# ShunyaoWang/quadruped_locomotion

Hardware: NVIDIA B200
Metric: contact-force QPs solved/sec (higher is better)
Workload: dtype f64

## Files before the change

### quadruped_locomotion_b200/csrc/qlb_api.cu

```cuda
#include <cuda_runtime.h>
#include <dlfcn.h>
#include <nccl.h>

#include <cmath>
#include <cstdio>
#include <cstdlib>
#include <cstring>
#include <mutex>
#include <new>

#include "qlb.h"
#include "qlb_aux.cuh"
#include "qlb_gen.cuh"
#include "qlb_qp_dense.cuh"
#include "qlb_records.cuh"
#include "qlb_solve.cuh"
#include "qlb_solve_quad.cuh"
#include "qlb_solve_fused.cuh"
#include "qlb_solve_single.cuh"
#include "qlb_swing.cuh"
#include "qlb_tick.cuh"

using namespace qlb;

// ... 141 lines not shown
    }
    const double* R3 = m->rot[l][3];
    const double* c3 = legs[l].link_com[3];
    for (int a = 0; a < 3; a++) m->com[l][3][a] = R3[3 * a] * c3[0] + R3[3 * a + 1] * c3[1] + R3[3 * a + 2] * c3[2];
    double acc = 0.0;
    for (int j = 3; j >= 0; j--) { acc += legs[l].link_mass[j]; m->msuf[l][j] = acc; }
  }
}

void build_device_params(const qlb_params* p, DeviceParams* d) {
  std::memset(d, 0, sizeof *d);
  for (int i = 0; i < 6; i++) d->S[i] = p->wrench_weights[i];
  d->W = p->ground_force_weight;
  d->fmin = p->min_normal_force > 0.0 ? p->min_normal_force : 0.0;
  d->mu_default = p->friction_default;
  d->gravity = p->gravity;
  d->tol = p->ipm_tolerance;
  d->max_iter = p->ipm_max_iterations;
  for (int i = 0; i < 3; i++) {
    d->kp_t[i] = p->kp_translation[i]; d->kd_t[i] = p->kd_translation[i]; d->kff_t[i] = p->kff_translation[i];
    d->kp_r[i] = p->kp_rotation[i]; d->kd_r[i] = p->kd_rotation[i]; d->kff_r[i] = p->kff_rotation[i];
    d->com[i] = p->com_in_base[i];
  }
  d->torso_mass = p->torso_mass;
  for (int l = 0; l < 4; l++) {
    d->leg_mass[l] = p->leg_mass[l];
    for (int a = 0; a < 3; a++) d->leg_pos[l][a] = p->leg_base_position[l][a];
  }
  d->grav_pct = p->gravity_compensation_percentage;
}

void narrow_model(const DeviceModel& m, DeviceModelT<float>* f) {
  const double* src = reinterpret_cast<const double*>(&m);
  float* dst = reinterpret_cast<float*>(f);
  for (size_t i = 0; i < sizeof(DeviceModel) / sizeof(double); i++) dst[i] = (float)src[i];
}
void narrow_params(const DeviceParams& d, DeviceParamsT<float>* f) {
  std::memset(f, 0, sizeof *f);
  for (int i = 0; i < 6; i++) f->S[i] = (float)d.S[i];
  f->W = (float)d.W; f->fmin = (float)d.fmin; f->mu_default = (float)d.mu_default; f->gravity = (float)d.gravity;
  f->tol = (float)d.tol; f->max_iter = d.max_iter;
  for (int i = 0; i < 3; i++) {
    f->kp_t[i] = (float)d.kp_t[i]; f->kd_t[i] = (float)d.kd_t[i]; f->kff_t[i] = (float)d.kff_t[i];
    f->kp_r[i] = (float)d.kp_r[i]; f->kd_r[i] = (float)d.kd_r[i]; f->kff_r[i] = (float)d.kff_r[i];
    f->com[i] = (float)d.com[i];
  }
  f->torso_mass = (float)d.torso_mass;
  for (int l = 0; l < 4; l++) {
    f->leg_mass[l] = (float)d.leg_mass[l];
    for (int a = 0; a < 3; a++) f->leg_pos[l][a] = (float)d.leg_pos[l][a];
  }
  f->grav_pct = (float)d.grav_pct;
}

bool params_ok(const qlb_params* p) {
  const double lo = 1e-12, hi = 1e12;
  if (!(p->ground_force_weight >= lo && p->ground_force_weight <= hi) || !(p->ipm_tolerance > 0.0) || p->ipm_max_iterations < 1)
    return false;
  for (int i = 0; i < 6; i++)
    if (!(p->wrench_weights[i] >= lo && p->wrench_weights[i] <= hi)) return false;
  if (!(p->friction_default >= 0.0) || !std::isfinite(p->friction_default)) return false;
  if (!(std::fabs(p->min_normal_force) <= 1e9)) return false;
  return std::isfinite(p->gravity);
}

bool aligned16(const void* p) { return (reinterpret_cast<uintptr_t>(p) & 15u) == 0; }

template <typename T>
int prepare_slot(qlb_context* ctx, SolveArgsT<T>& a, cudaStream_t st) {
  if (a.B > 0xFFFFFFF0ull) return QLB_ERR_BATCH_TOO_LARGE;
  int slot = -1;
  for (int i = 0; i < 8 && slot < 0; i++)
    if (cudaEventQuery(ctx->slot_done[i]) == cudaSuccess) slot = i;
  cudaGetLastError();
  if (slot < 0) slot = (int)(ctx->solve_calls % 8);
  ctx->solve_calls++;
  ctx->last_slot = slot;
  QLB_CUDA(ctx, cudaStreamWaitEvent(st, ctx->slot_done[slot], 0));
  a.counter = ctx->d_counter + 8 * slot;
  a.counter2 = a.counter + 1;
  a.counter3 = a.counter + 2;
  a.list_count = reinterpret_cast<unsigned*>(a.counter + 3);
  a.list2_count = reinterpret_cast<unsigned*>(a.counter + 4);
  QLB_CUDA(ctx, cudaMemsetAsync(a.counter, 0, 8 * sizeof(unsigned long long), st));
  if (ctx->list_cap < a.B) {
    const size_t cap = pow2_at_least(a.B, 1024);
    ctx->list_cap = 0;
    QLB_TRY(reserve(ctx, ctx->lists, 8 * 3 * cap * sizeof(unsigned)));
    ctx->list_cap = cap;
  }
  unsigned* list = reinterpret_cast<unsigned*>(ctx->lists.p) + (size_t)slot * 3 * ctx->list_cap;
  a.list = list;
  a.list2 = list + ctx->list_cap;
  a.list_pat = list + 2 * ctx->list_cap;
  return QLB_OK;
}

template <typename T, typename C>
constexpr int occ_index() { return sizeof(T) == 8 ? 0 : sizeof(C) == 8 ? 1 : 2; }

template <typename T, typename C, int MODE>
int launch_quad(qlb_context* ctx, SolveArgsT<T>& a, cudaStream_t st) {
  const SolveOccupancy& occ = ctx->occ[occ_index<T, C>()];
  const unsigned long long nb8 = (a.B + 7) / 8;
  const unsigned long long wantq = (nb8 + (kQuadThreads / 32) - 1) / (kQuadThreads / 32);
  const unsigned long long capq = (unsigned long long)ctx->sm_count * occ.quad[MODE];
  const unsigned long long capf = (unsigned long long)ctx->sm_count * occ.first[MODE];
  const unsigned gq = (unsigned)(wantq < capq ? wantq : capq);
  qlb_quad_first_kernel<T, C, MODE><<<(unsigned)(wantq < capf ? wantq : capf), kQuadThreads, 0, st>>>(a);
  QLB_CUDA(ctx, cudaGetLastError());
  ctx->launches++;
  qlb_quad_kernel<T, C, MODE, 1><<<gq, kQuadThreads, 0, st>>>(a);
  QLB_CUDA(ctx, cudaGetLastError());
  ctx->launches++;
  qlb_quad_kernel<T, C, MODE, 2><<<gq, kQuadThreads, 0, st>>>(a);
  QLB_CUDA(ctx, cudaGetLastError());
  ctx->launches++;
  QLB_CUDA(ctx, cudaEventRecord(ctx->slot_done[ctx->last_slot], st));
  return QLB_OK;
}

typedef CUresult (*EncodeTiledFn)(CUtensorMap*, CUtensorMapDataType, cuuint32_t, void*, const cuuint64_t*, const cuuint64_t*,
                                  const cuuint32_t*, const cuuint32_t*, CUtensorMapInterleave, CUtensorMapSwizzle,
                                  CUtensorMapL2promotion, CUtensorMapFloatOOBfill);
EncodeTiledFn encode_tiled_fn() {
  static EncodeTiledFn fn = []() -> EncodeTiledFn {
    void* p = nullptr;
    cudaDriverEntryPointQueryResult qres;
    if (cudaGetDriverEntryPoint("cuTensorMapEncodeTiled", &p, cudaEnableDefault, &qres) != cudaSuccess || qres != cudaDriverEntryPointSuccess) {
      cudaGetLastError();
      return nullptr;
    }
    return reinterpret_cast<EncodeTiledFn>(p);
  }();
  return fn;
}

template <typename T>
bool make_map(CUtensorMap* m, const T* ptr, unsigned long long B, int rows) {
  EncodeTiledFn fn = encode_tiled_fn();
  if (!fn) return false;
  const cuuint64_t gdim[2] = {(cuuint64_t)B, (cuuint64_t)rows};
  const cuuint64_t gstride[1] = {(cuuint64_t)B * sizeof(T)};
  const cuuint32_t box[2] = {8u * QLB_SUPER, (cuuint32_t)rows};
  const cuuint32_t estr[2] = {1u, 1u};
  return fn(m, sizeof(T) == 8 ? CU_TENSOR_MAP_DATA_TYPE_FLOAT64 : CU_TENSOR_MAP_DATA_TYPE_FLOAT32, 2, const_cast<T*>(ptr), gdim,
            gstride, box, estr, CU_TENSOR_MAP_INTERLEAVE_NONE, CU_TENSOR_MAP_SWIZZLE_NONE, CU_TENSOR_MAP_L2_PROMOTION_L2_128B,
            CU_TENSOR_MAP_FLOAT_OOB_FILL_NONE) == CUDA_SUCCESS;
}

bool make_mask_map(CUtensorMap* m, const uint8_t* ptr, unsigned long long B, int cols) {
  EncodeTiledFn fn = encode_tiled_fn();
  if (!fn) return false;
  const cuuint64_t gdim[1] = {(cuuint64_t)B};
  const cuuint64_t gstride[1] = {0};
  const cuuint32_t box[1] = {(cuuint32_t)cols};
  const cuuint32_t estr[1] = {1u};
  return fn(m, CU_TENSOR_MAP_DATA_TYPE_UINT8, 1, const_cast<uint8_t*>(ptr), gdim, gstride, box, estr, CU_TENSOR_MAP_INTERLEAVE_NONE,
            CU_TENSOR_MAP_SWIZZLE_NONE, CU_TENSOR_MAP_L2_PROMOTION_NONE, CU_TENSOR_MAP_FLOAT_OOB_FILL_NONE) == CUDA_SUCCESS;
}

template <typename T, typename C, int MODE>
int launch_single(qlb_context* ctx, SolveArgsT<T>& a, cudaStream_t st) {
  const SolveOccupancy& occ = ctx->occ[occ_index<T, C>()];
  using SG = Staging<T, MODE, QLB_SUPER>;
  using FL = FusedLayout<T, C, MODE, QLB_SUPER>;
  const T* src[SG::kNumSeg];
  for (int s = 0; s < SG::kNumSeg; s++) src[s] = SG::source(a, s);
  bool tma = a.B >= 64 && a.B < 0x7fffff00ull && ((a.B * sizeof(T)) % 16 == 0);
  for (int s = 0; s < SG::kNumSeg && tma; s++)
    if (src[s] && !aligned16(src[s])) tma = false;
  FusedMaps maps;
  std::memset(&maps, 0, sizeof maps);
  for (int s = 0; s < SG::kNumSeg && tma; s++)
    if (src[s] && !make_map<T>(&maps.seg[s], src[s], a.B, SG::rows(s))) tma = false;
  if (tma && (SG::kCols < 16 || !aligned16(a.mask) || !make_mask_map(&maps.mask, a.mask, a.B, SG::kCols))) tma = false;
  const unsigned long long ntiles = (a.B + 7) / 8;
  const unsigned long long want = (ntiles + kFusedWarps - 1) / kFusedWarps;
  int bps = occ.single[MODE][tma ? 1 : 0];
  if (ctx->fused_bps_cap > 0 && bps > ctx->fused_bps_cap) bps = ctx->fused_bps_cap;
  const unsigned long long cap = (unsigned long long)ctx->sm_count * bps;
  const unsigned grid = (unsigned)(want < cap ? want : cap);
  if (tma) qlb_single_kernel<T, C, MODE, QLB_SUPER, true><<<grid, kFusedThreads, FL::kTotal, st>>>(a, maps);
  else qlb_single_kernel<T, C, MODE, QLB_SUPER, false><<<grid, kFusedThreads, FL::kTotal, st>>>(a, maps);
  QLB_CUDA(ctx, cudaGetLastError());
  ctx->launches++;
  const unsigned long long capq = (unsigned long long)ctx->sm_count * occ.quad[MODE];
  const unsigned long long wantq = (ntiles + 3) / 4;
  qlb_quad_kernel<T, C, MODE, 2><<<(unsigned)(wantq < capq ? wantq : capq), kQuadThreads, 0, st>>>(a);
  QLB_CUDA(ctx, cudaGetLastError());
  ctx->launches++;
  QLB_CUDA(ctx, cudaEventRecord(ctx->slot_done[ctx->last_slot], st));
  return QLB_OK;
}

template <typename T, typename C>
bool query_occupancy(qlb_context* ctx) {
  SolveOccupancy& o = ctx->occ[occ_index<T, C>()];
  if (cudaOccupancyMaxActiveBlocksPerMultiprocessor(&o.quad[0], qlb_quad_kernel<T, C, 0, 2>, kQuadThreads, 0) != cudaSuccess ||
      cudaOccupancyMaxActiveBlocksPerMultiprocessor(&o.quad[1], qlb_quad_kernel<T, C, 1, 2>, kQuadThreads, 0) != cudaSuccess ||
      cudaOccupancyMaxActiveBlocksPerMultiprocessor(&o.first[0], qlb_quad_first_kernel<T, C, 0>, kQuadThreads, 0) != cudaSuccess ||
      cudaOccupancyMaxActiveBlocksPerMultiprocessor(&o.first[1], qlb_quad_first_kernel<T, C, 1>, kQuadThreads, 0) != cudaSuccess)
    return false;
  return o.quad[0] >= 1 && o.quad[1] >= 1 && o.first[0] >= 1 && o.first[1] >= 1;
}

template <typename T, int MODE>
bool prepare_single_kernels(qlb_context* ctx) {
  using C = double;
  using FL = FusedLayout<T, C, MODE, QLB_SUPER>;
  int* out = ctx->occ[occ_index<T, C>()].single[MODE];
  if (cudaFuncSetAttribute(qlb_single_kernel<T, C, MODE, QLB_SUPER, false>, cudaFuncAttributeMaxDynamicSharedMemorySize, FL::kTotal) != cudaSuccess ||
      cudaFuncSetAttribute(qlb_single_kernel<T, C, MODE, QLB_SUPER, true>, cudaFuncAttributeMaxDynamicSharedMemorySize, FL::kTotal) != cudaSuccess ||
      cudaFuncSetAttribute(qlb_single_kernel<T, C, MODE, QLB_SUPER, false>, cudaFuncAttributePreferredSharedMemoryCarveout, cudaSharedmemCarveoutMaxShared) != cudaSuccess ||
      cudaFuncSetAttribute(qlb_single_kernel<T, C, MODE, QLB_SUPER, true>, cudaFuncAttributePreferredSharedMemoryCarveout, cudaSharedmemCarveoutMaxShared) != cudaSuccess)
    return false;
  if (cudaOccupancyMaxActiveBlocksPerMultiprocessor(&out[0], qlb_single_kernel<T, C, MODE, QLB_SUPER, false>, kFusedThreads, FL::kTotal) != cudaSuccess ||
      cudaOccupancyMaxActiveBlocksPerMultiprocessor(&out[1], qlb_single_kernel<T, C, MODE, QLB_SUPER, true>, kFusedThreads, FL::kTotal) != cudaSuccess)
    return false;
  return out[0] >= 1 && out[1] >= 1;
}

template <typename T, int MODE>
int launch_solve(qlb_context* ctx, SolveArgsT<T>& a, cudaStream_t st) {
  QLB_TRY(prepare_slot(ctx, a, st));
  if constexpr (sizeof(T) == 4) {
    if (ctx->f32_pure) return launch_quad<float, float, MODE>(ctx, a, st);
  }
  if (ctx->pipeline == QLB_PIPELINE_FUSED) return launch_single<T, double, MODE>(ctx, a, st);
  return launch_quad<T, double, MODE>(ctx, a, st);
}

constexpr size_t kSoaBytesPerState = (kHostInRows + kHostOutRows) * sizeof(double) + sizeof(uint32_t) + 1;
struct SoaSlot {
  double* in;
  double* out;
  uint32_t* flags;
  uint8_t* mask;
};
SoaSlot soa_slot(const qlb_context* ctx, int slot) {
  const size_t cap = ctx->cap;
  double* in = reinterpret_cast<double*>(ctx->soa.p);
  double* out = in + kPipe * cap * kHostInRows;
  uint32_t* flags = reinterpret_cast<uint32_t*>(out + kPipe * cap * kHostOutRows);
  uint8_t* mask = reinterpret_cast<uint8_t*>(flags + kPipe * cap);
  return {in + slot * cap * kHostInRows, out + slot * cap * kHostOutRows, flags + slot * cap, mask + slot * cap};
}

int reserve_soa(qlb_context* ctx, size_t B) {
  if (B > kChunk) B = kChunk;
  if (B <= ctx->cap) return QLB_OK;
  const size_t cap = pow2_at_least(B, ctx->cap ? ctx->cap : 1024);
  ctx->cap = 0;
  QLB_TRY(reserve(ctx, ctx->soa, kPipe * cap * kSoaBytesPerState));
  ctx->cap = cap;
  return QLB_OK;
}

template <typename F>
int for_chunks(qlb_context* ctx, size_t B, size_t chunk, bool pipelined, F&& body) {
  cudaStream_t* streams = pipelined ? ctx->pipe : &ctx->stream;
  const int nstreams = pipelined ? kPipe : 1;
  int used = 0, rc = QLB_OK;
  for (size_t b0 = 0, i = 0; b0 < B && rc == QLB_OK; b0 += chunk, i++) {
    const int slot = (int)(i % nstreams);
    if (used <= slot) {
      used = slot + 1;
      const cudaError_t e = cudaStreamWaitEvent(streams[slot], ctx->soa_free, 0);
      if (e != cudaSuccess) { rc = cuda_fail(ctx, e, "cudaStreamWaitEvent"); break; }
    }
    rc = body(b0, B - b0 < chunk ? B - b0 : chunk, slot, streams[slot]);
  }
// ... 141 lines not shown
  while (*c) {
    const char* eol = c;
    while (*eol && *eol != '\n') eol++;
    int indent = 0;
    const char* t = c;
    while (t < eol && *t == ' ') { indent++; t++; }
    const char* hash = t;
    while (hash < eol && *hash != '#') hash++;
    const char* end = hash;
    while (end > t && (end[-1] == ' ' || end[-1] == '\t' || end[-1] == '\r')) end--;
    if (end > t && *t != '-') {
      const char* colon = t;
      while (colon < end && *colon != ':') colon++;
      if (colon < end) {
        while (depth > 0 && stack[depth - 1].indent >= indent) depth--;
        plen = depth > 0 ? stack[depth - 1].len : 0;
        const size_t klen = (size_t)(colon - t);
        if (plen + 1 + klen + 1 < sizeof path && depth < 32) {
          path[plen] = '/';
          std::memcpy(path + plen + 1, t, klen);
          const size_t nlen = plen + 1 + klen;
          path[nlen] = 0;
          const char* v = colon + 1;
          while (v < end && *v == ' ') v++;
          if (v < end) {
            char buf[64];
            const size_t vl = (size_t)(end - v) < sizeof buf - 1 ? (size_t)(end - v) : sizeof buf - 1;
            std::memcpy(buf, v, vl);
            buf[vl] = 0;
            char* stop = nullptr;
            const double val = std::strtod(buf, &stop);
            if (stop != buf) {
              const int k = qlb_params_set_key(p, path, val);
              if (k >= 0) seen[k] = true;
            }
          } else {
            stack[depth].indent = indent; stack[depth].len = nlen; depth++;
          }
        }
      }
    }
    c = *eol ? eol + 1 : eol;
  }
  int found = 0;
  const char* miss = nullptr;
  for (int k = 0; k < kNumParamKeys; k++) {
    if (seen[k]) found++;
    else if (!miss) miss = kParamKeys[k].path;
  }
  if (first_missing) *first_missing = miss;
  return found;
}

int qlb_create(qlb_context** out, const qlb_leg_model legs[QLB_NUM_LEGS], const qlb_params* params, int device,
               size_t max_batch) {
  if (!out || !legs) return QLB_ERR_INVALID_ARGUMENT;
  *out = nullptr;
  qlb_params defaults;
  qlb_default_params(&defaults);
  const qlb_params* p = params ? params : &defaults;
  if (!params_ok(p)) return QLB_ERR_INVALID_ARGUMENT;
  int ndev = 0;
  if (cudaGetDeviceCount(&ndev) != cudaSuccess || device < 0 || device >= ndev) {
    cudaGetLastError();
    return QLB_ERR_CUDA;
  }
  qlb_context* ctx = new (std::nothrow) qlb_context();
  if (!ctx) return QLB_ERR_ALLOC;
  ctx->device = device;
  ctx->params = *p;
  std::memcpy(ctx->legs, legs, sizeof ctx->legs);
  DeviceGuard guard(device);
  cudaDeviceProp prop;
  cudaError_t e = cudaGetDeviceProperties(&prop, device);
  if (e != cudaSuccess) { delete ctx; return QLB_ERR_CUDA; }
  ctx->sm_count = prop.multiProcessorCount;
  auto fail = [&](int code) { qlb_destroy(ctx); return code; };
  if (cudaMalloc(&ctx->d_model, sizeof(DeviceModel)) != cudaSuccess || cudaMalloc(&ctx->d_params, sizeof(DeviceParams)) != cudaSuccess ||
      cudaMalloc(&ctx->d_model_f, sizeof(DeviceModelT<float>)) != cudaSuccess ||
      cudaMalloc(&ctx->d_params_f, sizeof(DeviceParamsT<float>)) != cudaSuccess ||
      cudaMalloc(&ctx->d_counter, 64 * sizeof(unsigned long long)) != cudaSuccess ||
      cudaMalloc(&ctx->d_stats, QLB_STATS_NUM * sizeof(double)) != cudaSuccess)
    return fail(QLB_ERR_ALLOC);
  if (cudaStreamCreateWithFlags(&ctx->stream, cudaStreamNonBlocking) != cudaSuccess) return fail(QLB_ERR_CUDA);
  for (int i = 0; i < kPipe; i++)
    if (cudaStreamCreateWithFlags(&ctx->pipe[i], cudaStreamNonBlocking) != cudaSuccess) return fail(QLB_ERR_CUDA);
  for (int i = 0; i < 8; i++)
    if (cudaEventCreateWithFlags(&ctx->slot_done[i], cudaEventDisableTiming) != cudaSuccess) return fail(QLB_ERR_CUDA);
  if (cudaEventCreateWithFlags(&ctx->soa_free, cudaEventDisableTiming) != cudaSuccess) return fail(QLB_ERR_CUDA);
  DeviceModel hm;
  build_device_model(legs, &hm);
  if (cudaMemcpy(ctx->d_model, &hm, sizeof hm, cudaMemcpyHostToDevice) != cudaSuccess) return fail(QLB_ERR_CUDA);
  DeviceModelT<float> hmf;
  narrow_model(hm, &hmf);
  if (cudaMemcpy(ctx->d_model_f, &hmf, sizeof hmf, cudaMemcpyHostToDevice) != cudaSuccess) return fail(QLB_ERR_CUDA);
  if (qlb_set_params(ctx, p) != QLB_OK) return fail(QLB_ERR_CUDA);
  if (!query_occupancy<double, double>(ctx) || !query_occupancy<float, float>(ctx) || !query_occupancy<float, double>(ctx) ||
      !prepare_single_kernels<double, 0>(ctx) || !prepare_single_kernels<double, 1>(ctx) ||
      !prepare_single_kernels<float, 0>(ctx) || !prepare_single_kernels<float, 1>(ctx)) {
    cudaGetLastError();
    return fail(QLB_ERR_CUDA);
  }
  if (const char* e = std::getenv("QLB_FUSED_BPS")) ctx->fused_bps_cap = std::atoi(e);
  if (max_batch > 0 && reserve_soa(ctx, max_batch) != QLB_OK) return fail(QLB_ERR_ALLOC);
  *out = ctx;
  return QLB_OK;
}

int qlb_destroy(qlb_context* ctx) {
  if (!ctx) return QLB_OK;
  DeviceGuard guard(ctx->device);
  if (ctx->stream) { cudaStreamSynchronize(ctx->stream); cudaStreamDestroy(ctx->stream); }
  for (int i = 0; i < kPipe; i++)
    if (ctx->pipe[i]) { cudaStreamSynchronize(ctx->pipe[i]); cudaStreamDestroy(ctx->pipe[i]); }
  cudaFree(ctx->d_model); cudaFree(ctx->d_params); cudaFree(ctx->d_counter); cudaFree(ctx->d_stats);
  cudaFree(ctx->d_model_f); cudaFree(ctx->d_params_f); cudaFree(ctx->d_limb); cudaFree(ctx->d_limb_f);
  for (DeviceBuffer* b : {&ctx->lists, &ctx->soa, &ctx->rec, &ctx->prev, &ctx->qp}) cudaFree(b->p);
  for (int i = 0; i < 8; i++)
    if (ctx->slot_done[i]) cudaEventDestroy(ctx->slot_done[i]);
  if (ctx->soa_free) cudaEventDestroy(ctx->soa_free);
  cudaGetLastError();
  delete ctx;
  return QLB_OK;
}

int qlb_set_params(qlb_context* ctx, const qlb_params* params) {
  QLB_GUARD(ctx);
  if (!ctx || !params) return QLB_ERR_INVALID_ARGUMENT;
  if (!params_ok(params)) return QLB_ERR_INVALID_ARGUMENT;
  DeviceGuard guard(ctx->device);
  DeviceParams hp;
  build_device_params(params, &hp);
  QLB_CUDA(ctx, cudaDeviceSynchronize());
  QLB_CUDA(ctx, cudaMemcpy(ctx->d_params, &hp, sizeof hp, cudaMemcpyHostToDevice));
  DeviceParamsT<float> hpf;
  narrow_params(hp, &hpf);
  QLB_CUDA(ctx, cudaMemcpy(ctx->d_params_f, &hpf, sizeof hpf, cudaMemcpyHostToDevice));
  ctx->params = *params;
  return QLB_OK;
}

int qlb_get_params(const qlb_context* ctx, qlb_params* params) {
  if (!ctx || !params) return QLB_ERR_INVALID_ARGUMENT;
  *params = ctx->params;
  return QLB_OK;
}

int qlb_set_f32_core(qlb_context* ctx, int core) {
  QLB_GUARD(ctx);
  if (!ctx) return QLB_ERR_NOT_INITIALISED;
  if (core != QLB_F32_CORE_FP32 && core != QLB_F32_CORE_FP64) return QLB_ERR_INVALID_ARGUMENT;
  ctx->f32_pure = (core == QLB_F32_CORE_FP32);
  return QLB_OK;
}

int qlb_set_pipeline(qlb_context* ctx, int pipeline) {
  QLB_GUARD(ctx);
  if (!ctx) return QLB_ERR_NOT_INITIALISED;
  if (pipeline != QLB_PIPELINE_FUSED && pipeline != QLB_PIPELINE_THREE_PASS) return QLB_ERR_INVALID_ARGUMENT;
  ctx->pipeline = pipeline;
  return QLB_OK;
}

uint64_t qlb_launch_count(const qlb_context* ctx) { return ctx ? ctx->launches : 0; }

extern "C++" {
// ... 517 lines not shown
  if (B == 0) return QLB_OK;
  if (!G || !g0 || !x || !status || (p > 0 && (!CE || !ce0)) || (m > 0 && (!CI || !ci0))) return QLB_ERR_INVALID_ARGUMENT;
  DeviceGuard guard(ctx->device);
  if (host) {
    const size_t nin = (size_t)(n * n + n + n * p + p + n * m + m) * B, nout = (size_t)(n + 1) * B;
    QLB_TRY(reserve(ctx, ctx->qp, pow2_at_least((nin + nout) * sizeof(double) + 2 * B * sizeof(uint32_t), 4096)));
    double* dG = reinterpret_cast<double*>(ctx->qp.p); double* dg = dG + (size_t)n * n * B; double* dCE = dg + (size_t)n * B;
    double* dce = dCE + (size_t)n * p * B; double* dCI = dce + (size_t)p * B; double* dci = dCI + (size_t)n * m * B;
    double* d_out = dG + nin;
    uint32_t* d_u = reinterpret_cast<uint32_t*>(d_out + nout);
    if (p == 0) CE = ce0 = nullptr;
    if (m == 0) CI = ci0 = nullptr;
    return for_chunks(ctx, B, B, false, [&](size_t, size_t, int, cudaStream_t st) -> int {
      QLB_TRY(rows_to_device(ctx, dG, G, (size_t)n * n, 0, B, B, st));
      QLB_TRY(rows_to_device(ctx, dg, g0, n, 0, B, B, st));
      QLB_TRY(rows_to_device(ctx, dCE, CE, (size_t)n * p, 0, B, B, st));
      QLB_TRY(rows_to_device(ctx, dce, ce0, p, 0, B, B, st));
      QLB_TRY(rows_to_device(ctx, dCI, CI, (size_t)n * m, 0, B, B, st));
      QLB_TRY(rows_to_device(ctx, dci, ci0, m, 0, B, B, st));
      QLB_TRY(qp_dense(ctx, B, n, m, p, dG, dg, p ? dCE : nullptr, p ? dce : nullptr, m ? dCI : nullptr, m ? dci : nullptr,
                       d_out, d_out + (size_t)n * B, d_u, d_u + B, st, false));
      QLB_TRY(rows_to_host(ctx, x, d_out, n, 0, B, B, st));
      QLB_TRY(rows_to_host(ctx, cost, d_out + (size_t)n * B, 1, 0, B, B, st));
      QLB_TRY(rows_to_host(ctx, status, d_u, 1, 0, B, B, st));
      return rows_to_host(ctx, active, d_u + B, 1, 0, B, B, st);
    });
  }
  QpDenseArgs a;
  a.B = B; a.n = n; a.m = m; a.p = p; a.G = G; a.g0 = g0; a.CE = CE; a.ce0 = ce0; a.CI = CI; a.ci0 = ci0;
  a.x = x; a.cost = cost; a.status = status; a.active = active;
  unsigned long long blocks = (B + kQpWarpsPerCta - 1) / kQpWarpsPerCta;
  const unsigned long long cap = (unsigned long long)ctx->sm_count * 8ull;
  if (blocks > cap) blocks = cap;
  qlb_qp_dense_kernel<<<(unsigned)blocks, 32 * kQpWarpsPerCta, 0, static_cast<cudaStream_t>(stream)>>>(a);
  QLB_CUDA(ctx, cudaGetLastError());
  ctx->launches++;
  return QLB_OK;
}
}
}

int qlb_qp_dense(qlb_context* ctx, size_t B, int n, int m, int p, const double* G, const double* g0, const double* CE,
                 const double* ce0, const double* CI, const double* ci0, double* x, double* cost, uint32_t* status,
                 uint32_t* active, void* stream) {
  QLB_GUARD(ctx);
  return qp_dense(ctx, B, n, m, p, G, g0, CE, ce0, CI, ci0, x, cost, status, active, stream, false);
}

int qlb_qp_dense_host(qlb_context* ctx, size_t B, int n, int m, int p, const double* G, const double* g0,
                      const double* CE, const double* ce0, const double* CI, const double* ci0, double* x, double* cost,
                      uint32_t* status, uint32_t* active) {
  QLB_GUARD(ctx);
  return qp_dense(ctx, B, n, m, p, G, g0, CE, ce0, CI, ci0, x, cost, status, active, nullptr, true);
}

int qlb_measure_fp64_peak(qlb_context* ctx, double* tflops_out) {
  QLB_GUARD(ctx);
  if (!ctx || !tflops_out) return QLB_ERR_INVALID_ARGUMENT;
  DeviceGuard guard(ctx->device);
  cudaStream_t st = ctx->stream;
  cudaEvent_t e0, e1;
  QLB_CUDA(ctx, cudaEventCreate(&e0));
  QLB_CUDA(ctx, cudaEventCreate(&e1));
  const int iters = 4096, threads = 256;
  const int blocks = ctx->sm_count * 8;
  double best = 0.0;
  for (int rep = 0; rep < 5; rep++) {
    QLB_CUDA(ctx, cudaEventRecord(e0, st));
    qlb_fp64_peak_kernel<<<blocks, threads, 0, st>>>(ctx->d_stats, iters, 1.0 + rep);
    QLB_CUDA(ctx, cudaGetLastError());
    QLB_CUDA(ctx, cudaEventRecord(e1, st));
    QLB_CUDA(ctx, cudaEventSynchronize(e1));
    float ms = 0.f;
    QLB_CUDA(ctx, cudaEventElapsedTime(&ms, e0, e1));
    const double flops = 2.0 * 8.0 * 16.0 * (double)iters * (double)threads * (double)blocks;
    const double tf = flops / (ms * 1e-3) * 1e-12;
    if (rep > 0 && tf > best) best = tf;
  }
  cudaEventDestroy(e0);
  cudaEventDestroy(e1);
  *tflops_out = best;
  return QLB_OK;
}

}

struct qlb_controller {
  qlb_context* ctx = nullptr;
  size_t B = 0;
  qlb_tick_params p;
  int head = 0;
  cudaEvent_t reset_done = nullptr;
  uint8_t* limb = nullptr;
  uint8_t* refill = nullptr;
  double* efforts = nullptr;
  double* ring = nullptr;
  uint8_t* stance = nullptr;
  double* tau = nullptr;
  double* grf = nullptr;
};

namespace {

template <typename T>
int controller_tick(qlb_controller* c, size_t n, size_t b0, const T* q, const T* qd, const T* pose, const T* twist,
                    const T* tpose, const T* ttwist, const uint8_t* desired, const uint8_t* footstep, const uint8_t* contact,
                    const T* phase, const T* mu, const T* normals, const T* ptarget, const T* vtarget, T* command,
                    uint32_t* flags, T* grf, cudaStream_t st) {
  qlb_context* ctx = c->ctx;
  const size_t ld = c->B;
  T* tau = reinterpret_cast<T*>(c->tau);
  TickArgsT<T> a;
  std::memset(&a, 0, sizeof a);
  a.n = n; a.ld = ld; a.head = c->head;
  a.desired = desired; a.footstep = footstep; a.contact = contact; a.phase = phase; a.qd = qd;
  a.limb = c->limb + b0; a.refill = c->refill + b0; a.ring = c->ring + b0; a.stance = c->stance;
  a.flags = flags; a.tau = tau; a.efforts = c->efforts + b0; a.command = command; a.limit = c->p.effort_limit;
  fill_swing<T>(a.swing, ctx, c->p.swing, n, q, qd, ptarget, vtarget, nullptr);
  a.swing.qd_front = c->ring + (size_t)((c->head + 1) % kTickRing) * 12 * ld + b0; a.swing.ld_front = ld;
  a.swing.inv_window = (T)(1.0 / (10.0 * c->p.period));
  QLB_CUDA(ctx, cudaStreamWaitEvent(st, c->reset_done, 0));
  QLB_TRY(launch_items(ctx, n, 256, st, qlb_tick_prologue_kernel<T>, a));
  QLB_TRY(solve_state_t<T>(ctx, n, q, pose, twist, tpose, ttwist, c->stance, mu, normals, grf ? grf : reinterpret_cast<T*>(c->grf),
                           tau, flags, nullptr, nullptr, st, false));
  return launch_items(ctx, 4ull * n, 128, st, qlb_tick_epilogue_kernel<T>, a);
}

template <typename T>
int controller_update_t(qlb_controller* c, const T* q, const T* qd, const T* base_pose, const T* base_twist,
                        const T* target_pose, const T* target_twist, const uint8_t* desired_stance_mask,
                        const uint8_t* footstep_mask, const uint8_t* contact_mask, const T* phase, const T* mu,
                        const T* normals_world, const T* foot_target_position, const T* foot_target_velocity, T* command,
                        uint32_t* flags, T* grf, void* stream, bool host) {
  if (!c) return QLB_ERR_NOT_INITIALISED;
  QLB_GUARD(c->ctx);
  if (!c->ctx || !c->ctx->have_limb) return QLB_ERR_NOT_INITIALISED;
  if (!q || !qd || !base_pose || !base_twist || !target_pose || !target_twist || !desired_stance_mask || !contact_mask ||
      !phase || !command || !flags)
    return QLB_ERR_INVALID_ARGUMENT;
  qlb_context* ctx = c->ctx;
  DeviceGuard guard(ctx->device);
  const size_t B = c->B;
  int rc;
  if (!host) {
    rc = controller_tick<T>(c, B, 0, q, qd, base_pose, base_twist, target_pose, target_twist, desired_stance_mask, footstep_mask,
                            contact_mask, phase, mu, normals_world, foot_target_position, foot_target_velocity, command, flags,
                            grf, static_cast<cudaStream_t>(stream));
  } else {
    QLB_TRY(reserve_soa(ctx, B));
    const size_t cap = ctx->cap;
    const SoaSlot s = soa_slot(ctx, 0);
    constexpr int kIn = 11, kOut = 2;
    const T* src[kIn] = {q, qd, base_pose, base_twist, target_pose, target_twist, phase, mu, normals_world,
                         foot_target_position, foot_target_velocity};
    const int rows[kIn] = {12, 12, 7, 6, 7, 6, 4, 4, 12, 12, 12};
    static_assert(kPipe * kHostInRows >= 94 && kPipe * kHostOutRows >= 24 && kPipe >= 3, "staging too small for a tick");
    const uint8_t* msrc[3] = {desired_stance_mask, footstep_mask, contact_mask};
    T* const dst_out[kOut] = {command, grf};
    T* const dout[kOut] = {reinterpret_cast<T*>(s.out), reinterpret_cast<T*>(s.out) + 12 * cap};
    rc = for_chunks(ctx, B, cap, false, [&](size_t b0, size_t n, int, cudaStream_t st) -> int {
      const T* din[kIn];
      T* d = reinterpret_cast<T*>(s.in);
      for (int k = 0; k < kIn; d += (size_t)rows[k] * cap, k++) {
        din[k] = src[k] ? d : nullptr;
        QLB_TRY(rows_to_device(ctx, d, src[k], rows[k], b0, n, B, st));
      }
// ... 149 lines not shown
```

### quadruped_locomotion_b200/csrc/qlb_solve.cuh

```cuda
#pragma once

#include "qlb_device.cuh"

namespace qlb {

constexpr int kModePolish = 0, kModeIpm = 1, kModeDone = 2;
constexpr int kPolishPasses = 10;
constexpr double kNeighbourhood = 1e-3;

template <typename T>
struct SolveArgsT {
  unsigned long long B;
  const T* q;
  const T* quat;
  const T* wrench;
  const uint8_t* mask;
  const T* mu;
  const T* normals;
  const T* pose;
  const T* twist;
  const T* tpose;
  const T* ttwist;
  T* grf;
  T* tau;
  uint32_t* flags;
  T* netwrench;
  T* wrench_out;
  unsigned long long* counter;
  unsigned long long* counter2;
  unsigned* list;
  unsigned* list_pat;
  unsigned* list_count;
  unsigned long long* counter3;
  unsigned* list2;
  unsigned* list2_count;
  const DeviceModelT<T>* model;
  const DeviceParamsT<T>* params;
  const DeviceParamsT<double>* params64;
};
using SolveArgs = SolveArgsT<double>;

template <typename T>
__device__ __forceinline__ void quat_rel_log(const T* qt, const T* q, T (&v)[3]) {
  const T aw = qt[0], ax = -qt[1], ay = -qt[2], az = -qt[3];
  T w = aw * q[0] - ax * q[1] - ay * q[2] - az * q[3];
  T x = aw * q[1] + ax * q[0] + ay * q[3] - az * q[2];
  T y = aw * q[2] - ax * q[3] + ay * q[0] + az * q[1];
  T z = aw * q[3] + ax * q[2] - ay * q[1] + az * q[0];
  if (w < T(0.0)) { w = -w; x = -x; y = -y; z = -z; }
  const T n = sqrt(x * x + y * y + z * z);
  T k = T(2.0);
  if (n >= T(1e-12)) k = T(2.0) * atan2(n, w) / n;
  v[0] = k * x; v[1] = k * y; v[2] = k * z;
}

}
```

### quadruped_locomotion_b200/csrc/qlb_solve_quad.cuh

```cuda
#pragma once

#include "qlb_solve.cuh"

namespace qlb {

#ifndef QLB_POLISH_MU
#define QLB_POLISH_MU 1e-5f
#define QLB_POLISH_MIN_IT 2
#endif
#ifndef QLB_PDAS_ROUNDS
#define QLB_PDAS_ROUNDS 4
#endif
#ifndef QLB_IPM_MIN_CTAS
#define QLB_IPM_MIN_CTAS 3
#endif
#ifndef QLB_QUAD_MIN_CTAS
#define QLB_QUAD_MIN_CTAS 3
#endif
#ifndef QLB_FIRST_MIN_CTAS
#define QLB_FIRST_MIN_CTAS 3
#endif
constexpr int kQuadThreads = 128;

__device__ __forceinline__ float quad_max(float v) {
// ... 1168 lines not shown
  const unsigned pat0 = (STAGE == 1 && valid) ? (pat_word >> (5 * leg)) & 31u : 0u;
  quad_solve<creal, STAGE, kRescue>(L, cc, leg, quad, true, pat0, y, a0, sg1, sg2, status, it, defer);
  if (kRescue && STAGE == 2) {
    const bool again = (status == 2 || status == 3 || (status == 4 && !L.qbad));
    if (__any_sync(kFull, again)) {
      LegSetup<double> Ld;
      widen_setup(L, Ld);
      double yd[3];
      int a0d, sg1d, sg2d, statusd, itd;
      bool deferd;
      quad_solve<double, 0, false>(Ld, cc64, leg, quad, again, 0u, yd, a0d, sg1d, sg2d, statusd, itd, deferd);
      if (again) {
        y[0] = (creal)yd[0]; y[1] = (creal)yd[1]; y[2] = (creal)yd[2];
        a0 = a0d; sg1 = sg1d; sg2 = sg2d; status = statusd; it = itd;
      }
    }
  }
  if (STAGE == 1) {
    const unsigned hm = __ballot_sync(kFull, defer && valid && leg == 0);
    if (hm != 0u) {
      unsigned base = 0;
      if (lane == 0) base = atomicAdd(a.list2_count, __popc(hm));
      base = __shfl_sync(kFull, base, 0);
      if (defer && valid && leg == 0) a.list2[base + __popc(hm & ((1u << lane) - 1u))] = (unsigned)bq;
    }
  }
  quad_output<real, creal, real>(a, L, y, a0, sg1, sg2, status, it, bq, valid && !defer, leg, &jg[0][threadIdx.x], kQuadThreads);
}

template <typename real, typename creal, int MODE, int STAGE>
__global__ void __launch_bounds__(kQuadThreads, STAGE == 1 ? QLB_QUAD_MIN_CTAS : QLB_IPM_MIN_CTAS) qlb_quad_kernel(const SolveArgsT<real> a) {
  __shared__ DeviceParamsT<real> prm;
  __shared__ CoreConst<creal> cc;
  __shared__ CoreConst<double> cc64;
  __shared__ real jg[12][kQuadThreads];
  if (STAGE != 0 && __ldcg(STAGE == 1 ? a.list_count : a.list2_count) == 0u) return;
  {
    const uint32_t* src = reinterpret_cast<const uint32_t*>(a.params);
    uint32_t* dst = reinterpret_cast<uint32_t*>(&prm);
    for (int i = threadIdx.x; i < (int)(sizeof(DeviceParamsT<real>) / 4); i += blockDim.x) dst[i] = src[i];
    cc.load(a.params64);
    load_model_to_smem(a.model);
    if (Tol<creal>::rescue && STAGE == 2) cc64.load(a.params64);
  }
  __syncthreads();
  const int lane = threadIdx.x & 31;
  const int leg = lane & 3, quad = lane >> 2;
  const unsigned long long total = (STAGE == 0) ? a.B : (unsigned long long)(*(STAGE == 1 ? a.list_count : a.list2_count));
  unsigned long long* const work = (STAGE == 0) ? a.counter : (STAGE == 1 ? a.counter2 : a.counter3);
  const unsigned long long nbatch = (STAGE == 2) ? total : (total + 7) / 8;
  const unsigned long long B = a.B;
  const unsigned* const in_list = (STAGE == 1) ? a.list : a.list2;
  auto claim = [&]() {
    unsigned long long b = 0;
    if (lane == 0) b = atomicAdd(work, 1ull);
    return __shfl_sync(kFull, b, 0);
  };
  auto fetch = [&](const unsigned long long b, unsigned long long& idx, unsigned& pat, bool& ok) {
    const unsigned long long slot = (STAGE == 2) ? b : b * 8 + quad;
    ok = (b < nbatch) && (slot < total) && (STAGE != 2 || quad == 0);
    idx = B - 1; pat = 0u;
    if (ok) {
      idx = (STAGE == 0) ? slot : (unsigned long long)__ldcg(in_list + slot);
      if (STAGE == 1) pat = __ldcg(a.list_pat + slot);
    }
  };
  unsigned long long b0 = claim(), b1 = claim();
  unsigned long long idx0, idx1;
  unsigned pat0w, pat1w;
  bool ok0, ok1;
  fetch(b0, idx0, pat0w, ok0);
  fetch(b1, idx1, pat1w, ok1);
  while (b0 < nbatch) {
    const unsigned long long b2 = claim();
    unsigned long long idx2;
    unsigned pat2w;
    bool ok2;
    fetch(b2, idx2, pat2w, ok2);
    if (b1 < nbatch) quad_prefetch<real, MODE>(a, idx1, leg);
    quad_batch<real, creal, MODE, STAGE>(a, prm, cc, cc64, jg, idx0, pat0w, ok0, lane, leg, quad);
    b0 = b1; idx0 = idx1; pat0w = pat1w; ok0 = ok1;
    b1 = b2; idx1 = idx2; pat1w = pat2w; ok1 = ok2;
  }
}

}
```

### quadruped_locomotion_b200/csrc/qlb_solve_single.cuh

```cuda
#pragma once

#include "qlb_solve_fused.cuh"

namespace qlb {

#ifndef QLB_FUSED_MIN_CTAS
#define QLB_FUSED_MIN_CTAS 1
#endif
#ifndef QLB_FUSED_MIN_CTAS_F32
#define QLB_FUSED_MIN_CTAS_F32 1
#endif
#ifndef QLB_FUSED_THREADS
#define QLB_FUSED_THREADS 384
#endif
#ifndef QLB_DYNAMIC_PART
#define QLB_DYNAMIC_PART 4
#endif
#ifndef QLB_STASH_CAP
#define QLB_STASH_CAP 22
#endif
#ifndef QLB_ROUND_LOW
#define QLB_ROUND_LOW 8
#endif
constexpr int kFusedThreads = QLB_FUSED_THREADS;
constexpr int kFusedWarps = kFusedThreads / 32;
template <typename real> constexpr int fused_min_ctas() { return sizeof(real) == 4 ? QLB_FUSED_MIN_CTAS_F32 : QLB_FUSED_MIN_CTAS; }
template <typename real> constexpr int fused_smem_budget() { return (228 / fused_min_ctas<real>() - 1) * 1024; }

constexpr int kStashLane = 16;
constexpr int kSlFoot = 6, kSlMu = 9, kSlY = 10, kSlU = 13;
template <typename real, typename creal, int CAP>
struct StashLayout {
  static constexpr int kQ = 4 * CAP;
  static constexpr int kLaneBytes = kStashLane * kQ * (int)sizeof(creal);
  static constexpr int kJBytes = 12 * kQ * (int)sizeof(real);
  static constexpr int kBBytes = 6 * CAP * (int)sizeof(creal);
  static constexpr int kHBytes = 4 * CAP * 4;
  static constexpr int kBytes = ((kLaneBytes + kJBytes + kBBytes + kHBytes) + 15) & ~15;
};

template <typename real, typename creal, int MODE, int SUPER>
struct FusedLayout {
  static constexpr int kCtlWords = 8;
  static constexpr int kBarBytes = (kFusedWarps * 8 + 63) & ~63;
  static constexpr int kFixed = ((((int)sizeof(DeviceParamsT<real>) + 15) & ~15) + (((int)sizeof(CoreConst<creal>) + 15) & ~15) + kBarBytes +
                                 kFusedWarps * kCtlWords * 4 + 127) & ~127;
  static constexpr int kStatic = (int)sizeof(DeviceModelT<double>) + 128;
  static constexpr int kStage = Staging<real, MODE, SUPER>::kBytes;
  static constexpr int stash_bytes(int c) {
    return ((kStashLane * 4 * c * (int)sizeof(creal) + 12 * 4 * c * (int)sizeof(real) + 6 * c * (int)sizeof(creal) + 16 * c) + 15) & ~15;
  }
  static constexpr int warp_bytes(int c) { return (kStage + stash_bytes(c) + 127) & ~127; }
  static constexpr int cap_for(int c) { return (kStatic + kFixed + kFusedWarps * warp_bytes(c) <= fused_smem_budget<real>() || c <= 8) ? c : cap_for(c - 1); }
  static constexpr int kCap = cap_for(QLB_STASH_CAP);
  static_assert(kCap >= 10, "stash too small");
  static_assert(stash_bytes(kCap) == StashLayout<real, creal, kCap>::kBytes, "layout mismatch");
  static constexpr int kWarpBytes = warp_bytes(kCap);
  static constexpr int kTotal = kFixed + kFusedWarps * kWarpBytes;
  static_assert(kStatic + kTotal <= fused_smem_budget<real>(), "shared memory budget");
};

template <typename real, typename creal, int CAP>
struct WarpStash {
  creal* sl;
  real* sj;
  creal* sb;
  uint32_t* sh;
  __device__ WarpStash(unsigned char* base) {
    using SL = StashLayout<real, creal, CAP>;
    sl = reinterpret_cast<creal*>(base);
    sj = reinterpret_cast<real*>(base + SL::kLaneBytes);
    sb = reinterpret_cast<creal*>(base + SL::kLaneBytes + SL::kJBytes);
    sh = reinterpret_cast<uint32_t*>(base + SL::kLaneBytes + SL::kJBytes + SL::kBBytes);
  }
};


template <typename real, typename creal, int CAP>
__device__ __forceinline__ void stash_load(const WarpStash<real, creal, CAP>& ws, const int slot, const int leg, RoundState<creal>& q) {
  constexpr int Q = 4 * CAP;
  const int e = 4 * slot + leg;
  const uint32_t w1 = ws.sh[CAP + slot];
  q.idx = ws.sh[slot];
  q.gscale = __uint_as_float(ws.sh[2 * CAP + slot]);
  q.mask = w1 & 0xFu;
  q.alive = (w1 >> leg) & 1u;
  q.rounds = (int)(w1 >> 24);
  const unsigned pat = (w1 >> (4 + 5 * leg)) & 31u;
  q.a0 = (int)(pat & 1u);
  q.sg1 = ((pat >> 1) & 3u) == 1u ? -1 : (((pat >> 1) & 3u) == 2u ? 1 : 0);
  q.sg2 = ((pat >> 3) & 3u) == 1u ? -1 : (((pat >> 3) & 3u) == 2u ? 1 : 0);
  creal foot[3];
#pragma unroll
  for (int c = 0; c < 3; c++) {
    q.At[0][c] = ws.sl[c * Q + e];
    q.At[1][c] = ws.sl[(3 + c) * Q + e];
    foot[c] = ws.sl[(kSlFoot + c) * Q + e];
  }
  {
    creal t2[3];
    t2[0] = q.At[0][1] * q.At[1][2] - q.At[0][2] * q.At[1][1];
    t2[1] = q.At[0][2] * q.At[1][0] - q.At[0][0] * q.At[1][2];
    t2[2] = q.At[0][0] * q.At[1][1] - q.At[0][1] * q.At[1][0];
    const creal rn = q.alive ? fast_rsqrt(t2[0] * t2[0] + t2[1] * t2[1] + t2[2] * t2[2]) : creal(0.0);
#pragma unroll
// ... 39 lines not shown
#pragma unroll
    for (int r = 0; r < 6; r++) q.At[c][r] = creal(0.0);
    q.y[c] = creal(0.0); q.u[c] = creal(0.0);
  }
  q.mu = creal(0.0); q.a0 = 0; q.sg1 = 0; q.sg2 = 0; q.gscale = 1.f; q.mask = 0u; q.alive = false; q.rounds = 0; q.idx = 0u;
  int slot = nth_set_bit(unassigned, quad);
  bool active = slot >= 0;
  {
    const int ntake = min(8, __popc(unassigned));
#pragma unroll 1
    for (int i = 0; i < ntake; i++) unassigned &= unassigned - 1u;
  }
  bool fresh = active;
#pragma unroll 1
  for (;;) {
    if (fresh) stash_load(ws, slot, leg, q);
    fresh = false;
    bool done, fail;
    const int bslot = active ? slot : 0;
    dbas_round<creal>(q, ws.sb + bslot, CAP, cc, leg, active, done, fail);
    const bool leave = active && (done || fail);
    if (__any_sync(kFull, leave)) {
      LegSetup<creal> L;
#pragma unroll
      for (int c = 0; c < 3; c++) {
#pragma unroll
        for (int r = 0; r < 6; r++) L.At[c][r] = q.At[c][r];
      }
      L.alive = q.alive; L.mask = q.mask;
      const int oslot = active ? slot : 0;
      quad_output<real, creal, real>(a, L, q.y, q.a0, q.sg1, q.sg2, 0, q.rounds, (unsigned long long)q.idx, active && done, leg,
                               ws.sj + 4 * oslot + leg, Q);
      const unsigned fm = __ballot_sync(kFull, active && fail && leg == 0);
      if (fm != 0u) {
        unsigned base = 0;
        if (lane == 0) base = atomicAdd(a.list2_count, __popc(fm));
        base = __shfl_sync(kFull, base, 0);
        if (active && fail && leg == 0) a.list2[base + __popc(fm & ((1u << lane) - 1u))] = q.idx;
      }
      const unsigned freed = __reduce_or_sync(kFull, leave ? (1u << slot) : 0u);
      occ &= ~freed;
      const unsigned wm = __ballot_sync(kFull, leave && leg == 0);
      const int rank = __popc(wm & ((1u << (lane & ~3)) - 1u));
      __syncwarp();
      if (leave) {
        slot = nth_set_bit(unassigned, rank);
        active = slot >= 0;
        fresh = active;
      }
      {
        const int ntake = min(__popc(wm), __popc(unassigned));
#pragma unroll 1
        for (int i = 0; i < ntake; i++) unassigned &= unassigned - 1u;
      }
    }
    const int nact = __popc(__ballot_sync(kFull, active && leg == 0));
    if (nact == 0) break;
    if (!final && nact + __popc(unassigned) < run_min) {
      stash_save(ws, active ? slot : 0, leg, q, active && !fresh);
      break;
    }
  }
  __syncwarp();
}

template <typename real, typename creal, int MODE, int SUPER, bool TMA>
__global__ void __launch_bounds__(kFusedThreads, fused_min_ctas<real>())
qlb_single_kernel(const SolveArgsT<real> a, const __grid_constant__ FusedMaps maps) {
  using FL = FusedLayout<real, creal, MODE, SUPER>;
  constexpr int CAP = FL::kCap;
  constexpr int Q = 4 * CAP;
  constexpr int kRunMin = CAP - 7;
  constexpr int kRunLow = QLB_ROUND_LOW < kRunMin ? QLB_ROUND_LOW : kRunMin;
  constexpr int kCols = 8 * SUPER;
  extern __shared__ __align__(128) unsigned char smem[];
  DeviceParamsT<real>& prm = *reinterpret_cast<DeviceParamsT<real>*>(smem);
  CoreConst<creal>& cc = *reinterpret_cast<CoreConst<creal>*>(smem + ((sizeof(DeviceParamsT<real>) + 15) & ~15));
  static_assert(((sizeof(DeviceParamsT<real>) + 15) & ~15) + sizeof(CoreConst<creal>) + FL::kBarBytes + kFusedWarps * FL::kCtlWords * 4 <= FL::kFixed, "fixed part");
  unsigned long long* bars = reinterpret_cast<unsigned long long*>(smem + FL::kFixed - FL::kBarBytes);
  volatile unsigned* ctl = reinterpret_cast<volatile unsigned*>(smem + FL::kFixed - FL::kBarBytes - kFusedWarps * FL::kCtlWords * 4) +
                           (threadIdx.x >> 5) * FL::kCtlWords;
  const int warp = threadIdx.x >> 5, lane = threadIdx.x & 31;
  const int leg = lane & 3, quad = lane >> 2;
  unsigned char* wbase = smem + FL::kFixed + warp * FL::kWarpBytes;
  unsigned char* stage = wbase;
  const WarpStash<real, creal, CAP> ws(wbase + FL::kStage);
  const uint32_t bar = smem_u32(&bars[warp]);
  {
    const uint32_t* src = reinterpret_cast<const uint32_t*>(a.params);
    uint32_t* dst = reinterpret_cast<uint32_t*>(&prm);
    for (int i = threadIdx.x; i < (int)(sizeof(DeviceParamsT<real>) / 4); i += blockDim.x) dst[i] = src[i];
    cc.load(a.params64);
    load_model_to_smem(a.model);
    if (TMA && lane == 0) {
      mbar_init(bar, 1);
      asm volatile("fence.mbarrier_init.release.cluster;" ::: "memory");
      asm volatile("fence.proxy.async.shared::cta;" ::: "memory");
    }
  }
  __syncthreads();
  const unsigned nbox = (unsigned)((a.B + kCols - 1) / kCols);
  unsigned occ = 0u;

  const unsigned nwarps = gridDim.x * kFusedWarps;
  const unsigned gwarp = blockIdx.x * kFusedWarps + warp;
  const unsigned share = (nbox - nbox / QLB_DYNAMIC_PART) / nwarps;
  const unsigned dyn_base = share * nwarps;
  if (lane == 0) { ctl[0] = share; ctl[1] = dyn_base; ctl[2] = 0u; ctl[3] = nbox; ctl[4] = (unsigned)a.B; ctl[5] = 0u; ctl[6] = 0u; }
  __syncwarp();
  auto claim_raw = [&](const bool doit) -> unsigned {
    unsigned b = 0;
    if (lane == 0 && doit) b = atomicAdd(reinterpret_cast<unsigned*>(a.counter), 1u);
    return b;
  };
  unsigned pending_claim = claim_raw(share <= 1);
  unsigned cur;
  {
    cur = __shfl_sync(kFull, share > 0 ? gwarp : dyn_base + pending_claim, 0);
    if (share == 0) pending_claim = claim_raw(true);
  }
  if (cur < nbox) stage_issue<real, MODE, SUPER, TMA>(a, maps, cur, stage, bar, lane);
  if (lane == 0) ctl[5] = (cur < nbox) ? 0x200u : 0u;
  __syncwarp();
  unsigned nxt = 0;
#pragma unroll 1
  for (;;) {
    const unsigned cw = __shfl_sync(kFull, ctl[5], 0);
    const bool have = (cw & 0x200u) != 0u;
    if (have) {
      const int sub = (int)(cw & 0xffu);
      const unsigned cw_wait = (sub == 0 && TMA) ? (cw ^ 0x100u) : cw;
      if (sub + 1 < SUPER && lane == 0) ctl[5] = cw_wait + 1u;
      if (sub == 0) {
        if (TMA) mbar_wait(bar, (cw >> 8) & 1u);
        else { cp_async_wait_all(); __syncwarp(); }
      }
      const int col = sub * 8 + quad;
      const unsigned s0 = cur * kCols + col, Bu = ctl[4];
      const bool valid = s0 < Bu;
      const unsigned bq = valid ? s0 : (Bu - 1u);
      RawIn<real, MODE> in;
      stage_read<real, MODE, SUPER>(a, stage, prm.mu_default, leg, col, bq, in);
      if (!valid) in.mask = 0u;
      if (sub == SUPER - 1) {
        __syncwarp();
        const unsigned taken = __shfl_sync(kFull, ctl[2], 0) + 1u, shr = __shfl_sync(kFull, ctl[0], 0);
        if (lane == 0) ctl[2] = taken;
        nxt = __shfl_sync(kFull, taken < shr ? blockIdx.x * kFusedWarps + warp + taken * (gridDim.x * kFusedWarps) : ctl[1] + pending_claim, 0);
        pending_claim = claim_raw(taken + 1 >= shr);
        const bool more = nxt < __shfl_sync(kFull, ctl[3], 0);
        if (lane == 0) ctl[5] = (cw_wait & 0x100u) | (more ? 0x200u : 0u);
        if (more) stage_issue<real, MODE, SUPER, TMA>(a, maps, nxt, stage, bar, lane);
      }
      const int slot = nth_set_bit(~occ & ((1u << CAP) - 1u), quad);
      LegSetup<creal> L;
      quad_setup<real, MODE, creal>(a, prm, in, bq, valid, true, leg, L, ws.sj + 4 * slot + leg, Q);
      int status;
      creal y[3], t[6];
      bool hard;
      unsigned pat;
      quad_first_solve<real, creal>(L, cc.sinv, cc.winv, cc.fmin, leg, y, t, status, hard, pat);
      hard = hard && valid;
      creal net[6];
#pragma unroll
      for (int r = 0; r < 6; r++) net[r] = fma(-cc.sinv[r], t[r], L.b[r]);
      quad_output<real, creal, real>(a, L, y, 0, 0, 0, status, 0, bq, valid, leg, ws.sj + 4 * slot + leg, Q, net);
      if (hard) {
        const int e = 4 * slot + leg;
#pragma unroll
        for (int c = 0; c < 3; c++) {
#pragma unroll
          for (int k = 0; k < 2; k++) ws.sl[(3 * k + c) * Q + e] = L.At[k][c];
          ws.sl[(kSlFoot + c) * Q + e] = L.foot[c];
          ws.sl[(kSlY + c) * Q + e] = y[c];
          ws.sl[(kSlU + c) * Q + e] = creal(0.0);
        }
        ws.sl[kSlMu * Q + e] = L.mu;
        ws.sb[leg * CAP + slot] = sel4(leg, L.b[0], L.b[1], L.b[2], L.b[3]);
        if (leg < 2) ws.sb[(4 + leg) * CAP + slot] = (leg & 1) ? L.b[5] : L.b[4];
        if (leg == 0) {
          ws.sh[slot] = (unsigned)bq;
          ws.sh[CAP + slot] = L.mask | (pat << 4);
          ws.sh[2 * CAP + slot] = __float_as_uint(L.gscale);
        }
      }
      occ |= __reduce_or_sync(kFull, hard ? (1u << slot) : 0u);
      __syncwarp();
      if (sub + 1 == SUPER) cur = nxt;
    }
    const int pending = __popc(occ);
    if (have ? (pending >= kRunMin) : (pending > 0)) round_phase<real, creal, CAP>(a, cc, ws, occ, !have, kRunLow, lane, leg, quad);
    if (!have) break;
  }
}

}
```

Measured before the change: 2.357 billion.

## Reset work counters in-kernel via last-CTA instead of per-solve memset

Drops the per-call cudaMemsetAsync of the slot counters before the solve kernels. The last CTA to finish each kernel now resets the counters it consumed, using a done-counter atomic, and the quad path appends a trailing memset. The fused path's tail quad kernel is launched with exactly sm_count blocks instead of a computed grid. The aim is to remove a memset node from the launch sequence. In exchange every CTA does an extra syncthreads and atomic at exit, and correctness now depends on the counters being zeroed at context creation and every kernel completing normally. It also adds optional globaltimer phase-clock instrumentation behind a compile flag.

```diff
diff --git a/quadruped_locomotion_b200/csrc/qlb_api.cu b/quadruped_locomotion_b200/csrc/qlb_api.cu
--- a/quadruped_locomotion_b200/csrc/qlb_api.cu
+++ b/quadruped_locomotion_b200/csrc/qlb_api.cu
@@ -247,7 +247,7 @@
   a.counter3 = a.counter + 2;
   a.list_count = reinterpret_cast<unsigned*>(a.counter + 3);
   a.list2_count = reinterpret_cast<unsigned*>(a.counter + 4);
-  QLB_CUDA(ctx, cudaMemsetAsync(a.counter, 0, 8 * sizeof(unsigned long long), st));
+  a.done = reinterpret_cast<unsigned*>(a.counter + 5);
   if (ctx->list_cap < a.B) {
     const size_t cap = pow2_at_least(a.B, 1024);
     ctx->list_cap = 0;
@@ -281,6 +281,7 @@
   qlb_quad_kernel<T, C, MODE, 2><<<gq, kQuadThreads, 0, st>>>(a);
   QLB_CUDA(ctx, cudaGetLastError());
   ctx->launches++;
+  QLB_CUDA(ctx, cudaMemsetAsync(a.counter, 0, 8 * sizeof(unsigned long long), st));
   QLB_CUDA(ctx, cudaEventRecord(ctx->slot_done[ctx->last_slot], st));
   return QLB_OK;
 }
@@ -350,9 +351,7 @@
   else qlb_single_kernel<T, C, MODE, QLB_SUPER, false><<<grid, kFusedThreads, FL::kTotal, st>>>(a, maps);
   QLB_CUDA(ctx, cudaGetLastError());
   ctx->launches++;
-  const unsigned long long capq = (unsigned long long)ctx->sm_count * occ.quad[MODE];
-  const unsigned long long wantq = (ntiles + 3) / 4;
-  qlb_quad_kernel<T, C, MODE, 2><<<(unsigned)(wantq < capq ? wantq : capq), kQuadThreads, 0, st>>>(a);
+  qlb_quad_kernel<T, C, MODE, 2><<<(unsigned)ctx->sm_count, kQuadThreads, 0, st>>>(a);
   QLB_CUDA(ctx, cudaGetLastError());
   ctx->launches++;
   QLB_CUDA(ctx, cudaEventRecord(ctx->slot_done[ctx->last_slot], st));
@@ -660,6 +659,7 @@
       cudaMalloc(&ctx->d_counter, 64 * sizeof(unsigned long long)) != cudaSuccess ||
       cudaMalloc(&ctx->d_stats, QLB_STATS_NUM * sizeof(double)) != cudaSuccess)
     return fail(QLB_ERR_ALLOC);
+  if (cudaMemset(ctx->d_counter, 0, 64 * sizeof(unsigned long long)) != cudaSuccess) return fail(QLB_ERR_CUDA);
   if (cudaStreamCreateWithFlags(&ctx->stream, cudaStreamNonBlocking) != cudaSuccess) return fail(QLB_ERR_CUDA);
   for (int i = 0; i < kPipe; i++)
     if (cudaStreamCreateWithFlags(&ctx->pipe[i], cudaStreamNonBlocking) != cudaSuccess) return fail(QLB_ERR_CUDA);
@@ -1343,6 +1343,17 @@
   *tflops_out = best;
   return QLB_OK;
 }
+
+#ifdef QLB_PHASE_CLOCKS
+int qlb_phase_clocks_read(qlb_context* ctx, unsigned long long* out, unsigned nwarps) {
+  QLB_GUARD(ctx);
+  if (!ctx || !out || nwarps > kPhaseClockWarps) return QLB_ERR_INVALID_ARGUMENT;
+  DeviceGuard guard(ctx->device);
+  QLB_CUDA(ctx, cudaDeviceSynchronize());
+  QLB_CUDA(ctx, cudaMemcpyFromSymbol(out, qlb_phase_clocks, 8ull * nwarps * sizeof(unsigned long long)));
+  return QLB_OK;
+}
+#endif
 
 }
 
diff --git a/quadruped_locomotion_b200/csrc/qlb_solve.cuh b/quadruped_locomotion_b200/csrc/qlb_solve.cuh
--- a/quadruped_locomotion_b200/csrc/qlb_solve.cuh
+++ b/quadruped_locomotion_b200/csrc/qlb_solve.cuh
@@ -37,8 +37,22 @@
   const DeviceModelT<T>* model;
   const DeviceParamsT<T>* params;
   const DeviceParamsT<double>* params64;
+  unsigned* done;
 };
 using SolveArgs = SolveArgsT<double>;
+
+template <typename F>
+__device__ __forceinline__ void last_cta_resets(unsigned* done, F&& reset) {
+  __syncthreads();
+  if (threadIdx.x == 0) {
+    __threadfence();
+    if (atomicAdd(done, 1u) == gridDim.x - 1u) {
+      __threadfence();
+      reset();
+      *done = 0u;
+    }
+  }
+}
 
 template <typename T>
 __device__ __forceinline__ void quat_rel_log(const T* qt, const T* q, T (&v)[3]) {
diff --git a/quadruped_locomotion_b200/csrc/qlb_solve_quad.cuh b/quadruped_locomotion_b200/csrc/qlb_solve_quad.cuh
--- a/quadruped_locomotion_b200/csrc/qlb_solve_quad.cuh
+++ b/quadruped_locomotion_b200/csrc/qlb_solve_quad.cuh
@@ -1274,6 +1274,7 @@
     b0 = b1; idx0 = idx1; pat0w = pat1w; ok0 = ok1;
     b1 = b2; idx1 = idx2; pat1w = pat2w; ok1 = ok2;
   }
-}
-
-}
+  if (STAGE == 2) last_cta_resets(a.done, [&] { *a.counter3 = 0ull; *a.list2_count = 0u; });
+}
+
+}
diff --git a/quadruped_locomotion_b200/csrc/qlb_solve_single.cuh b/quadruped_locomotion_b200/csrc/qlb_solve_single.cuh
--- a/quadruped_locomotion_b200/csrc/qlb_solve_single.cuh
+++ b/quadruped_locomotion_b200/csrc/qlb_solve_single.cuh
@@ -21,6 +21,20 @@
 #endif
 #ifndef QLB_ROUND_LOW
 #define QLB_ROUND_LOW 8
+#endif
+#ifdef QLB_PHASE_CLOCKS
+constexpr unsigned kPhaseClockWarps = 8192;
+__device__ unsigned long long qlb_phase_clocks[8 * kPhaseClockWarps];
+__device__ __forceinline__ unsigned long long global_ns() {
+  unsigned long long t;
+  asm volatile("mov.u64 %0, %%globaltimer;" : "=l"(t));
+  return t;
+}
+__device__ __forceinline__ unsigned smid() {
+  unsigned s;
+  asm volatile("mov.u32 %0, %%smid;" : "=r"(s));
+  return s;
+}
 #endif
 constexpr int kFusedThreads = QLB_FUSED_THREADS;
 constexpr int kFusedWarps = kFusedThreads / 32;
@@ -226,6 +240,18 @@
                            (threadIdx.x >> 5) * FL::kCtlWords;
   const int warp = threadIdx.x >> 5, lane = threadIdx.x & 31;
   const int leg = lane & 3, quad = lane >> 2;
+#ifdef QLB_PHASE_CLOCKS
+  auto phase_clock = [&](const int k) {
+    const unsigned w = blockIdx.x * kFusedWarps + warp;
+    if (lane == 0 && w < kPhaseClockWarps) {
+      unsigned long long* r = qlb_phase_clocks + 8ull * w;
+      r[2 * k] = clock64();
+      r[2 * k + 1] = global_ns();
+      if (k == 0) { r[6] = smid(); r[7] = gridDim.x; }
+    }
+  };
+  phase_clock(0);
+#endif
   unsigned char* wbase = smem + FL::kFixed + warp * FL::kWarpBytes;
   unsigned char* stage = wbase;
   const WarpStash<real, creal, CAP> ws(wbase + FL::kStage);
@@ -333,9 +359,16 @@
       if (sub + 1 == SUPER) cur = nxt;
     }
     const int pending = __popc(occ);
+#ifdef QLB_PHASE_CLOCKS
+    if (!have) phase_clock(1);
+#endif
     if (have ? (pending >= kRunMin) : (pending > 0)) round_phase<real, creal, CAP>(a, cc, ws, occ, !have, kRunLow, lane, leg, quad);
     if (!have) break;
   }
-}
-
-}
+#ifdef QLB_PHASE_CLOCKS
+  phase_clock(2);
+#endif
+  last_cta_resets(a.done, [&] { *a.counter = 0ull; });
+}
+
+}
```

Result: no change. 2.371 billion, median of 6 (+0.6%).
